# dfdazac/mpqe

Measured on AMD Instinct MI355X. Metric: query-graphs/sec (encoder fwd+bwd), higher is better.
Workload: dtype f32; 1 GPU; AIFB-shaped full query mix: 11 batches x B=512 per step (1/2/3-chain, 2x each of 2-inter, 3-inter, 3-inter_chain, 3-chain_inter), embed_dim=128, readout=mp, adaptive=True, num_layers=3 unshared, KG aifb (2601 entities, 89 typed relations); parallelism=single GPU

## Files before the change

mpqe_amd/csrc/step_chain.h:

```cpp
#pragma once
#include <type_traits>
#include "gemm_core.h"

#define CH_GB 16
#define CH_FIRST 1
#define CH_LAST 2
#define CH_LEVEL_END 4
#define CH_RELU 8
#define CH_MASK 16
#define CH_NOSTORE 32
#define CH_ADDG 64
#define CH_NOBIAS 128
#define CH_TSLOT_ON (1 << 20)
#define CH_MASK_LEVELS 4
#define CH_MAX_OPS 80
#define CH_MAX_CV 12

typedef float f32x2 __attribute__((ext_vector_type(2)));
typedef const f32x2 __attribute__((address_space(1))) * gvec2_ptr;
__device__ __forceinline__ f32x2 gload2(const float *p) { return *(gvec2_ptr)(p); }

struct ChainOp {
    unsigned char src, node, layer, level;
    int mat, flags;
    int wt_slot;
    int aux;
    int pad;
};
struct ChainRef {
    int batch, g0, fwd_begin, fwd_count, bwd_begin, bwd_count;
    int tb;
    int done;
    int e0;
    int gi0;
    int B;
    unsigned meta;
    int rof;
};

template <int NCB>
struct WHalf {
    float v[4][4][NCB];
};
template <int NCB> struct chain_vec;
template <> struct chain_vec<1> { typedef float type; };
template <> struct chain_vec<2> { typedef f32x2 type; };
template <> struct chain_vec<4> { typedef f32x4 type; };
template <int NCB> struct chain_bits { typedef unsigned char type; };
template <> struct chain_bits<4> { typedef unsigned short type; };

template <int NCB>
__device__ __forceinline__ void chain_gload(float (&d)[NCB], const float *p) {
    if constexpr (NCB == 1) d[0] = gload1(p);
    else if constexpr (NCB == 2) {
        const f32x2 q = gload2(p);
        d[0] = q[0];
        d[1] = q[1];
    } else {
        const f32x4 q = gload4(p);
#pragma unroll
        for (int c = 0; c < NCB; ++c) d[c] = q[c & 3];
    }
}
template <int NCB>
__device__ __forceinline__ void chain_store(float *p, const float (&v)[NCB]) {
    typename chain_vec<NCB>::type q;
    if constexpr (NCB == 1) q = v[0];
    else {
#pragma unroll
        for (int c = 0; c < NCB; ++c) q[c] = v[c];
    }
    *reinterpret_cast<typename chain_vec<NCB>::type *>(p) = q;
}

template <int NCB>
__device__ __forceinline__ void chain_lload(float (&d)[NCB], const float *p) {
    const typename chain_vec<NCB>::type q = *reinterpret_cast<const typename chain_vec<NCB>::type *>(p);
    if constexpr (NCB == 1) d[0] = q;
    else {
#pragma unroll
        for (int c = 0; c < NCB; ++c) d[c] = q[c];
    }
}
__device__ __forceinline__ unsigned long long chain_gran_load(const unsigned long long *g) {
#ifdef MPQE_EMU
    return *g;
#else
    typedef unsigned long long __attribute__((address_space(1))) * gp_t;
    return __hip_atomic_load((gp_t)g, __ATOMIC_RELAXED, __HIP_MEMORY_SCOPE_AGENT);
#endif
}
__device__ __forceinline__ unsigned chain_count_load(const unsigned *p) {
#ifdef MPQE_EMU
    return *p;
#else
// ... 48 lines not shown
template <int OFF>
__device__ __forceinline__ float chain_row_ror(float v) {
#ifdef MPQE_EMU
    return __shfl_xor(v, OFF, 64);
#else
    return __int_as_float(__builtin_amdgcn_update_dpp(0, __float_as_int(v), 0x120 + OFF, 0xF, 0xF, false));
#endif
}
__device__ __forceinline__ float chain_sum16(float v) {
    v += chain_row_ror<8>(v);
    v += chain_row_ror<4>(v);
    v += chain_row_ror<2>(v);
    v += chain_row_ror<1>(v);
    return v;
}
__device__ __forceinline__ void chain_relu_push(float &v, unsigned &bits) {
#ifdef MPQE_EMU
    const bool p = v > 0.f;
    v = p ? v : 0.f;
    bits = (bits << 1) | (p ? 1u : 0u);
#else
    float o;
    asm volatile("v_cmp_lt_f32 vcc, 0, %2\n\tv_cndmask_b32 %0, 0, %2, vcc\n\tv_addc_co_u32 %1, vcc, %1, %1, vcc"
                 : "=&v"(o), "+v"(bits)
                 : "v"(v)
                 : "vcc");
    v = o;
#endif
}
__device__ __forceinline__ void chain_mask_pop(float &v, unsigned &bits) {
#ifdef MPQE_EMU
    const bool p = (bits >> 31) != 0u;
    bits <<= 1;
    v = p ? v : 0.f;
#else
    float o;
    asm volatile("v_add_co_u32 %1, vcc, %1, %1\n\tv_cndmask_b32 %0, 0, %2, vcc" : "=&v"(o), "+v"(bits) : "v"(v) : "vcc");
    v = o;
#endif
}

#ifndef CHAIN_ZERO_C
#define CHAIN_ZERO_C 1
#endif
#ifndef CHAIN_DBG
#define CHAIN_DBG 0
#endif
#ifndef CHAIN_LATE_DECODE
#define CHAIN_LATE_DECODE 1
#endif
#ifndef CHAIN_NOLOAD
#define CHAIN_NOLOAD 0
#endif
template <int NCB>
__device__ __forceinline__ void chain_load_t(WHalf<NCB> &f, const float *wp, int D, int t) {
    if (CHAIN_DBG == 1) return;
#pragma unroll
    for (int u = 0; u < 4; ++u) chain_gload<NCB>(f.v[t][u], wp + (long long)(16 * t + u) * D);
}

template <int NCB>
__device__ __forceinline__ void chain_mma(f32x4 (&acc)[NCB], const WHalf<NCB> &f, const float *xp) {
#pragma unroll
    for (int t = 0; t < 4; ++t) {
        const f32x4 a = *reinterpret_cast<const f32x4 *>(xp + 16 * t);
#pragma unroll
        for (int u = 0; u < 4; ++u)
#pragma unroll
            for (int c = 0; c < NCB; ++c)
                acc[c] = __builtin_amdgcn_mfma_f32_16x16x4f32(a[u], f.v[t][u][c], acc[c], 0, 0, 0);
    }
}

template <int NCB, int KS, int NW = 4>
struct ChainLds {
    static constexpr int D = 16 * NCB * NW / KS, LDX = D + 4, BUF = 4 * CH_GB * LDX, MT = 64 * NW / KS;
    float xs[2 * BUF];
    static constexpr int NCV = CH_MAX_CV;
    float cv[NCV * D];
    typename chain_bits<NCB>::type mbits[CH_MASK_LEVELS * 4 * MT];
    const float *rowp[4 * CH_GB + 2 * CH_GB];
    float *gradp[4 * CH_GB];
    float nrm[4 * CH_GB];
    const float *wp[CH_MAX_OPS];
    int opw[CH_MAX_OPS][2];
    int opp[CH_MAX_OPS];
    int cvid[NCV];
    int cvl[NCV];
    __device__ __forceinline__ float *red() { return cv; }
#if CHAIN_DBG == 6
    long long *trace;
    int trace_n;
#endif
};

template <int NCB, int KS, int NW>
__device__ __forceinline__ void chain_colsum(ChainLds<NCB, KS, NW> &S, const float *X, unsigned mask, int ng,
                                             float *__restrict__ dst) {
    constexpr int D = 16 * NCB * NW / KS, LDX = D + 4, NP = 256 / D;
    const int col = threadIdx.x % D, part = threadIdx.x / D;
    if (threadIdx.x < 256) {
        float s = 0.f;
        for (int n = 0; n < 4; ++n) {
            if (!((mask >> n) & 1u)) continue;
            for (int i = part; i < ng; i += NP) s += X[(n * CH_GB + i) * LDX + col];
        }
        S.red()[threadIdx.x] = s;
    }
    __syncthreads();
    if (threadIdx.x < D && dst) {
        float t = S.red()[threadIdx.x];
        for (int q = 1; q < NP; ++q) t += S.red()[threadIdx.x + q * D];
        dst[threadIdx.x] = t;
    }
    __syncthreads();
}
struct ChainStep {
    int src, node, tslot, level, flags, part;
};

template <int NCB, int KS, bool BWD, int NW, bool RO = false>
__device__ __forceinline__ void chain_run(ChainLds<NCB, KS, NW> &S, const int first_op, int T , int N, int ng,
                                          float *__restrict__ Xrows, long long level_stride, int &cur,
                                          float *parts = nullptr, int blk = 0,
                                          const unsigned long long *cv_gran = nullptr, unsigned cv_tag = 0,
                                          int32_t *cv_err = nullptr) {
    constexpr int D = 16 * NCB * NW / KS, LDX = D + 4, BUF = 4 * CH_GB * LDX;
    constexpr int CW = NW / KS;
    constexpr int IPO = D / KS / 64;
    constexpr int MT = 64 * NW / KS;
    const int lane = threadIdx.x & 63, wave = threadIdx.x >> 6;
    const int j = lane & 15, kq = lane >> 4;
    const int ks = wave / CW;
    const int kbase = ks * (D / KS);
    const int colb = (wave % CW) * 16 * NCB + NCB * j;
    const bool finisher = __builtin_amdgcn_readfirstlane(ks) == KS - 1;
    auto get_op = [&](int it) -> ChainStep {
        const int k = first_op + (it < T ? it : T - 1) / IPO;
        const int w = __builtin_amdgcn_readfirstlane(S.opw[k][0]);
        ChainStep o;
        o.src = w & 0xff;
        o.node = (w >> 8) & 0xff;
        o.tslot = RO ? (w >> 16) & 0xff : o.node;
        o.level = (w >> 24) & 0xff;
        o.flags = __builtin_amdgcn_readfirstlane(S.opw[k][1]);
        o.part = __builtin_amdgcn_readfirstlane(S.opp[k]);
        return o;
    };
    struct RawOp {
        int w0, w1, w2;
    };
    auto get_raw = [&](int it) -> RawOp {
        const int k = first_op + (it < T ? it : T - 1) / IPO;
        return RawOp{S.opw[k][0], S.opw[k][1], S.opp[k]};
    };
    auto decode = [&](const RawOp &r) -> ChainStep {
        const int w = __builtin_amdgcn_readfirstlane(r.w0);
        ChainStep o;
        o.src = w & 0xff;
        o.node = (w >> 8) & 0xff;
        o.tslot = RO ? (w >> 16) & 0xff : o.node;
        o.level = (w >> 24) & 0xff;
        o.flags = __builtin_amdgcn_readfirstlane(r.w1);
        o.part = __builtin_amdgcn_readfirstlane(r.w2);
        return o;
    };
    auto wptr = [&](int it) -> const float * {
        const int itc = it < T ? it : T - 1;
        const int h = itc % IPO;
        const float *W = S.wp[first_op + itc / IPO];
        return W + (long long)(kbase + 64 * h + 4 * kq) * D + colb;
    };
    f32x4 acc[NCB];
#if CHAIN_DBG == 6
    int trace_i = BWD ? 2048 : 0;
#endif
    float bs[NCB];
#pragma unroll
    for (int c = 0; c < NCB; ++c) bs[c] = 0.f;
    const float *pend_tile = nullptr;
    float *pend_out = nullptr;
    bool pend_on = false, pend_store = false;
    int pend_part = -1;
    auto flush_rows = [&]() {
        float l[4][NCB];
#pragma unroll
        for (int r = 0; r < 4; ++r) chain_lload<NCB>(l[r], pend_tile + r * LDX);
        if (BWD) {
#pragma unroll
            for (int c = 0; c < NCB; ++c) bs[c] = 0.f;
        }
        if (ng == CH_GB) {
            if (pend_store) {
#pragma unroll
                for (int r = 0; r < 4; ++r) chain_store<NCB>(pend_out + (long long)r * N * D, l[r]);
            }
            if (BWD) {
#pragma unroll
                for (int r = 0; r < 4; ++r)
#pragma unroll
                    for (int c = 0; c < NCB; ++c) bs[c] += l[r][c];
            }
        } else {
#pragma unroll
            for (int r = 0; r < 4; ++r)
                if (4 * kq + r < ng) {
                    if (pend_store) chain_store<NCB>(pend_out + (long long)r * N * D, l[r]);
                    if (BWD) {
#pragma unroll
                        for (int c = 0; c < NCB; ++c) bs[c] += l[r][c];
                    }
                }
        }
        if (BWD && pend_part >= 0) {
            float t[NCB];
#pragma unroll
            for (int c = 0; c < NCB; ++c) {
                t[c] = bs[c] + __shfl_xor(bs[c], 16, 64);
                t[c] += __shfl_xor(t[c], 32, 64);
            }
            if (kq == 0) chain_store<NCB>(parts + (long long)(pend_part + blk) * D + colb, t);
        }
        pend_on = false;
    };
    auto item = [&](const ChainStep &op, int it, WHalf<NCB> &f, WHalf<NCB> &fn, const float *wn, auto inplace_tag) {
        constexpr bool INPLACE = decltype(inplace_tag)::value;
        const int h = it % IPO;
#if CHAIN_DBG == 6
#define CHAIN_TRACE(tag)                                                                        \
    if (S.trace && (threadIdx.x & 127) == 0 && S.trace_n < 4000) {                              \
        const long long tt_ = (long long)__builtin_amdgcn_s_memtime();                          \
        __builtin_amdgcn_s_waitcnt(0xC07F);                                                     \
        S.trace[(threadIdx.x >> 7) * 4096 + S.trace_n * 0 + trace_i] = tt_ * 8 + (tag);         \
        ++trace_i;                                                                              \
    }
        CHAIN_TRACE(0)
#else
#define CHAIN_TRACE(tag)
#endif
        const float *xp = S.xs + cur * BUF + (op.src * CH_GB + j) * LDX + kbase + 64 * h + 4 * kq;
        unsigned long long ga[RO ? 4 : 1][RO ? (NCB + 1) / 2 : 1];
        if constexpr (RO) {
            if (finisher && h == IPO - 1 && (op.flags & CH_LAST) && (op.flags & CH_ADDG)) {
                const float *Xadd = Xrows + (long long)op.level * level_stride + ((long long)(4 * kq) * N + op.node) * D + colb;
#pragma unroll
                for (int r = 0; r < 4; ++r)
#pragma unroll
                    for (int c2 = 0; c2 < (NCB + 1) / 2; ++c2) {
                        const bool in = 4 * kq + r < ng;
                        if constexpr (NCB % 2 == 0)
                            ga[r][c2] = in ? chain_gran_load(reinterpret_cast<const unsigned long long *>(Xadd + (long long)r * N * D) + c2) : 0ull;
                        else
                            ga[r][c2] = in ? (unsigned long long)chain_count_load(reinterpret_cast<const unsigned *>(Xadd + (long long)r * N * D)) : 0ull;
                    }
            }
        }
        f32x4 av[4];
#pragma unroll
        for (int t = 0; t < 4; ++t) av[t] = *reinterpret_cast<const f32x4 *>(xp + 16 * t);
#pragma unroll
        for (int t = 0; t < 4; ++t) {
            const f32x4 a = av[t];
#pragma unroll
            for (int u = 0; u < 4; ++u) {
                if (CHAIN_DBG != 1 && !CHAIN_NOLOAD && !INPLACE) chain_gload<NCB>(fn.v[t][u], wn + (long long)(16 * t + u) * D);
                __builtin_amdgcn_sched_barrier(0);
#if CHAIN_DBG == 2
#pragma unroll
                for (int c = 0; c < NCB; ++c) asm volatile("" ::"v"(f.v[t][u][c]), "v"(a[u]));
#else
                if (CHAIN_ZERO_C && t == 0 && u == 0 && h == 0 && (op.flags & CH_FIRST)) {
#pragma unroll
                    for (int c = 0; c < NCB; ++c)
                        acc[c] = __builtin_amdgcn_mfma_f32_16x16x4f32(a[u], f.v[t][u][c], f32x4{0.f, 0.f, 0.f, 0.f}, 0, 0, 0);
                } else {
#pragma unroll
                    for (int c = 0; c < NCB; ++c)
                        acc[c] = __builtin_amdgcn_mfma_f32_16x16x4f32(a[u], f.v[t][u][c], acc[c], 0, 0, 0);
                }
#endif
                __builtin_amdgcn_sched_barrier(0);
                if (CHAIN_DBG != 1 && !CHAIN_NOLOAD && INPLACE) {
                    chain_gload<NCB>(f.v[t][u], wn + (long long)(16 * t + u) * D);
                    __builtin_amdgcn_sched_barrier(0);
                }
            }
        }
        CHAIN_TRACE(1)
        if (h != IPO - 1) return;
        if (op.flags & CH_LAST) {
            static_assert(KS <= 2, "the hand-off below is written for two K parts");
            float *Xn = S.xs + (cur ^ 1) * BUF;
            float *tile = Xn + (op.tslot * CH_GB + 4 * kq) * LDX + colb;
            if (KS > 1 && !finisher) {
#pragma unroll
                for (int r = 0; r < 4; ++r) {
                    float pv[NCB];
#pragma unroll
                    for (int c = 0; c < NCB; ++c) pv[c] = acc[c][r];
                    chain_store<NCB>(tile + r * LDX, pv);
                }
            }
            float v[4][NCB];
            float bv[NCB];
            if (finisher) {
#pragma unroll
                for (int r = 0; r < 4; ++r)
#pragma unroll
                    for (int c = 0; c < NCB; ++c) v[r][c] = acc[c][r];
                if (!BWD && KS == 1) chain_lload<NCB>(bv, S.cv + op.part * D + colb);
            }
            if (KS > 1) __syncthreads();
            if (KS > 1 && finisher && !BWD) chain_lload<NCB>(bv, S.cv + op.part * D + colb);
            if (KS > 1 && !finisher) {
                if (pend_on) flush_rows();
                pend_store = !(op.flags & CH_NOSTORE);
                pend_part = op.part;
                pend_on = pend_store || (BWD && pend_part >= 0);
                pend_tile = tile;
                pend_out = Xrows + (long long)op.level * level_stride + ((long long)(4 * kq) * N + op.node) * D + colb;
                if (!BWD && cv_gran) {
                    constexpr int NCVc = ChainLds<NCB, KS, NW>::NCV;
                    const int ns = op.part + 1;
                    if (ns < NCVc && (int)threadIdx.x < D) {
                        const int id = S.cvid[ns];
                        if (id >= 0) S.cv[ns * D + threadIdx.x] = chain_gran_read1(cv_gran + (long long)id * D + threadIdx.x, cv_tag, cv_err);
                    }
                }
            }
            CHAIN_TRACE(2)
            auto finish = [&](auto mode_tag) {
                constexpr int MODE = decltype(mode_tag)::value;
                if (KS > 1) {
                    float l[4][NCB];
#pragma unroll
                    for (int r = 0; r < 4; ++r) chain_lload<NCB>(l[r], tile + r * LDX);
#pragma unroll
                    for (int r = 0; r < 4; ++r)
#pragma unroll
                        for (int c = 0; c < NCB; ++c) v[r][c] += l[r][c];
                }
                CHAIN_TRACE(4)
                const int mslot = ((op.level - 1) * 4 + op.node) * MT + (threadIdx.x & (MT - 1));
                if (!BWD && !(RO && (op.flags & CH_NOBIAS))) {
#pragma unroll
                    for (int r = 0; r < 4; ++r)
#pragma unroll
                        for (int c = 0; c < NCB; ++c) v[r][c] += bv[c];
                }
                if constexpr (RO) {
                    if (op.flags & CH_ADDG) {
#pragma unroll
                        for (int r = 0; r < 4; ++r)
#pragma unroll
                            for (int c = 0; c < NCB; ++c)
                                v[r][c] += __uint_as_float((unsigned)(ga[r][c / 2] >> (32 * (c & 1))));
                    }
                }
                if (MODE == 1) {
                    unsigned bits = 0;
#pragma unroll
                    for (int r = 0; r < 4; ++r)
// ... 9 lines not shown
                }
                CHAIN_TRACE(5)
#pragma unroll
                for (int r = 0; r < 4; ++r) chain_store<NCB>(tile + r * LDX, v[r]);
                CHAIN_TRACE(6)
                const bool var_row = KS == 1 && BWD && op.part >= 0;
                if (var_row) {
#pragma unroll
                    for (int c = 0; c < NCB; ++c) bs[c] = 0.f;
                }
                float *Xout = Xrows + (long long)op.level * level_stride + ((long long)(4 * kq) * N + op.node) * D + colb;
                if (ng == CH_GB) {
                    if (KS == 1 && !(op.flags & CH_NOSTORE)) {
#pragma unroll
                        for (int r = 0; r < 4; ++r) chain_store<NCB>(Xout + (long long)r * N * D, v[r]);
                    }
                    if (BWD && KS == 1) {
#pragma unroll
                        for (int r = 0; r < 4; ++r)
#pragma unroll
                            for (int c = 0; c < NCB; ++c) bs[c] += v[r][c];
                    }
                } else {
#pragma unroll
                    for (int r = 0; r < 4; ++r) {
                        if (4 * kq + r < ng) {
                            if (KS == 1 && !(op.flags & CH_NOSTORE)) chain_store<NCB>(Xout + (long long)r * N * D, v[r]);
                            if (BWD && KS == 1) {
#pragma unroll
                                for (int c = 0; c < NCB; ++c) bs[c] += v[r][c];
                            }
                        }
                    }
                }
                CHAIN_TRACE(7)
                if (var_row) {
                    float t[NCB];
#pragma unroll
                    for (int c = 0; c < NCB; ++c) {
                        t[c] = bs[c] + __shfl_xor(bs[c], 16, 64);
                        t[c] += __shfl_xor(t[c], 32, 64);
                    }
                    if (kq == 0) chain_store<NCB>(parts + (long long)(op.part + blk) * D + colb, t);
                }
            };
            if (finisher) {
                if (!BWD && (op.flags & CH_RELU)) finish(std::integral_constant<int, 1>());
                else if (BWD && (op.flags & CH_MASK)) finish(std::integral_constant<int, 2>());
                else finish(std::integral_constant<int, 0>());
            }
            if (!CHAIN_ZERO_C) {
#pragma unroll
                for (int c = 0; c < NCB; ++c) acc[c] = f32x4{0.f, 0.f, 0.f, 0.f};
            }
        }
        CHAIN_TRACE(3)
        if (op.flags & CH_LEVEL_END) {
            __syncthreads();
            cur ^= 1;
            if (KS > 1 && !finisher) {
                if (pend_on) flush_rows();
            }
        }
    };
    if (T <= 0) return;
#pragma unroll
    for (int c = 0; c < NCB; ++c) acc[c] = f32x4{0.f, 0.f, 0.f, 0.f};

    ChainStep oc = get_op(0), on = get_op(1);
    int it = 0;
    if constexpr (KS == 2 && CHAIN_DBG != 5) {
        WHalf<NCB> f0;
#pragma unroll
        for (int t = 0; t < 4; ++t) chain_load_t<NCB>(f0, wptr(0), D, t);
        __builtin_amdgcn_sched_barrier(0);
        const float *wn1 = wptr(1);
        while (true) {
#if CHAIN_LATE_DECODE
            const RawOp r2_ = get_raw(it + 2);
            const float *w2_ = wptr(it + 2);
            item(oc, it, f0, f0, wn1, std::true_type());
            if (++it >= T) break;
            oc = on;
            on = decode(r2_);
            wn1 = w2_;
#else
            const ChainStep o2_ = get_op(it + 2);
            const float *w2_ = wptr(it + 2);
            item(oc, it, f0, f0, wn1, std::true_type());
            if (++it >= T) break;
            oc = on;
            on = o2_;
            wn1 = w2_;
#endif
        }
    } else if constexpr (NCB <= 2) {
        WHalf<NCB> f0, f1, f2, f3;
#pragma unroll
        for (int t = 0; t < 4; ++t) chain_load_t<NCB>(f0, wptr(0), D, t);
#pragma unroll
        for (int t = 0; t < 4; ++t) chain_load_t<NCB>(f1, wptr(1), D, t);
#pragma unroll
        for (int t = 0; t < 4; ++t) chain_load_t<NCB>(f2, wptr(2), D, t);
        __builtin_amdgcn_sched_barrier(0);
#define CHAIN_STEP(F, FN)                       \
    {                                           \
        const ChainStep o2_ = get_op(it + 2);   \
        item(oc, it, F, FN, wptr(it + 3), std::false_type());      \
        if (++it >= T) break;                   \
        oc = on;                                \
        on = o2_;                               \
    }
        while (true) {
            CHAIN_STEP(f0, f3)
            CHAIN_STEP(f1, f0)
            CHAIN_STEP(f2, f1)
            CHAIN_STEP(f3, f2)
        }
#undef CHAIN_STEP
    } else {
        WHalf<NCB> f0, f1, f2;
#pragma unroll
        for (int t = 0; t < 4; ++t) chain_load_t<NCB>(f0, wptr(0), D, t);
#pragma unroll
        for (int t = 0; t < 4; ++t) chain_load_t<NCB>(f1, wptr(1), D, t);
        __builtin_amdgcn_sched_barrier(0);
#define CHAIN_STEP(F, FN)                       \
    {                                           \
        const ChainStep o2_ = get_op(it + 2);   \
        item(oc, it, F, FN, wptr(it + 2), std::false_type());      \
        if (++it >= T) break;                   \
        oc = on;                                \
        on = o2_;                               \
    }
        while (true) {
            CHAIN_STEP(f0, f2)
            CHAIN_STEP(f1, f0)
            CHAIN_STEP(f2, f1)
        }
#undef CHAIN_STEP
    }
}

struct ChainArgs {
    const ChainRef *refs;
    const ChainOp *ops;
    const long long *node_map;
    long long map_len;
    const float *mode_emb;
    long long num_modes;
    const long long *anchor_ids, *targets, *negs;
    float *H, *GH;
    const float *WT;
    const float *VT;
    unsigned *epoch_f;
    float *DG;
    const int *erow;
    long long Manchor, Gtot;
    float *parts;
    float *block_terms;
    long long level_stride;
    float margin, eps;
    float *s_pos, *s_neg, *terms;
    float *q_out;
    int32_t *err;
    int backward;
    long long *stamps;
    int cb, nchain;
    const unsigned long long *cv_gran;
    const unsigned *epoch_b;
    const unsigned *wt_count;
    int wt_blocks;
    unsigned *done;
    unsigned *arrive;
    const int *done_inc;
    int wt_early;
    int ro;
    int ro_layer, ro_scatter;
};

__device__ __forceinline__ void chain_stamp(const ChainArgs &ca, int slot) {
#ifndef MPQE_EMU
    if (ca.stamps && threadIdx.x == 0) {
        ca.stamps[(long long)ca.cb * 8 + slot] = (long long)wall_clock64();
        if (slot == 0 || slot == 6) {
            const long long t = (long long)__builtin_amdgcn_s_memtime();
            __builtin_amdgcn_s_waitcnt(0xC07F);
            ca.stamps[((long long)ca.nchain + ca.cb) * 8 + (slot == 0 ? 0 : 1)] = t;
        }
    }
#endif
}
__device__ __forceinline__ void chain_stamp_where(const ChainArgs &ca, int batch, int fwd_ops) {
#ifndef MPQE_EMU
    if (ca.stamps && threadIdx.x == 0) {
        const unsigned hw = __builtin_amdgcn_s_getreg((31 << 11) | 4);
        const unsigned xcc = __builtin_amdgcn_s_getreg((3 << 11) | 20);
        ca.stamps[(long long)ca.cb * 8 + 7] = (long long)hw | ((long long)xcc << 32) | ((long long)batch << 40) |
                                                   ((long long)fwd_ops << 48);
    }
#endif
}

template <int NCB, int KS, int NW, bool RO = false>
__device__ __forceinline__ void chain_block(const StepDev *__restrict__ sd, const LayerPtrs &lp, const TablePtrs &tabs,
                                            const ChainArgs &ca, ChainLds<NCB, KS, NW> &S) {
    constexpr int D = 16 * NCB * NW / KS, LDX = D + 4, BUF = 4 * CH_GB * LDX;
    constexpr int DB = D / 64;
    constexpr int IPO = D / KS / 64;
    constexpr int LPR = D / 4;
    const int tid = threadIdx.x, lane = tid & 63, wave = tid >> 6;
    const bool four = NW == 4 || tid < 256;
    const ChainRef ref = ca.refs[ca.cb];
    if (ref.batch < 0) return;
    const BatchDev &b = sd->b[ref.batch];
    const int N = (int)(ref.meta & 15u), A = (int)((ref.meta >> 4) & 15u), L = b.L, g0 = ref.g0;
    const int ng = ref.B - g0 < CH_GB ? ref.B - g0 : CH_GB;
    const int nrows = ng * N;
    const long long row0 = b.row_off + (long long)g0 * N;
    const long long gi0 = b.g_off + g0;

    chain_stamp(ca, 0);
    chain_stamp_where(ca, ref.batch, ref.fwd_count);
#if CHAIN_DBG == 6
#ifndef CHAIN_TRACE_BATCH
#define CHAIN_TRACE_BATCH 0
#endif
    if (threadIdx.x == 0) {
        S.trace = (ca.stamps && ref.batch == CHAIN_TRACE_BATCH && g0 == 0) ? ca.stamps + (long long)ca.nchain * 16 : nullptr;
        S.trace_n = 0;
    }
#endif
#if CHAIN_DBG == 4
    for (int q = 0; q < (int)((blockIdx.x / 8) % 4) * 6; ++q) __builtin_amdgcn_s_sleep(127);
#endif
    const int rof = RO ? ref.rof : 0, nfwd = ref.fwd_count + rof;
    const int nops = nfwd + ref.bwd_count;
    ChainOp op;
    if (tid < nops) op = ca.ops[ref.fwd_begin + tid];
    if (tid < 4 * CH_GB + 2 * CH_GB) {
        const float *src = nullptr;
        float *gdst = nullptr;
        const int rN = (int)(ref.meta & 15u), rA = (int)((ref.meta >> 4) & 15u);
        if (tid < 4 * CH_GB) {
            const int i = tid / rN, n = tid - i * rN;
            if (tid < nrows) {
                if (n < rA) {
                    const int tab = (int)((ref.meta >> (8 + 4 * n)) & 15u);
                    const long long e = (long long)ref.e0 + (long long)n * ref.B + i;
                    long long row;
                    int er = -2;
                    if (ca.erow) er = ca.erow[e];
                    if (er == -2) row = table_row(ca.node_map, ca.map_len, ca.anchor_ids[e], tabs.rows[tab], ca.err);
                    else {
                        row = er;
                        if (er < 0) flag_error(ca.err, MPQE_FLAG_BAD_NODE_ID);
                    }
                    if (row >= 0) {
                        src = tabs.table[tab] + row * D;
                        if (tabs.grad[tab]) gdst = tabs.grad[tab] + row * D;
                    }
                } else {
                    const long long m = b.var_id[n - rA];
                    if (m < 0 || m >= ca.num_modes) flag_error(ca.err, MPQE_FLAG_BAD_NODE_ID);
                    else src = ca.mode_emb + m * D;
                }
            }
            S.gradp[tid] = gdst;
        } else {
            const int i = (tid - 4 * CH_GB) & (CH_GB - 1);
            const bool is_neg = tid >= 5 * CH_GB;
            if (i < ng) {
                const int tab = (int)((ref.meta >> 20) & 15u);
                const long long e = ca.Manchor + (is_neg ? ca.Gtot : 0) + ref.gi0 + i;
                long long row;
                int er = -2;
                if (ca.erow) er = ca.erow[e];
                if (er == -2)
                    row = table_row(ca.node_map, ca.map_len, is_neg ? ca.negs[ref.gi0 + i] : ca.targets[ref.gi0 + i],
                                    tabs.rows[tab], ca.err);
                else {
                    row = er;
                    if (er < 0) flag_error(ca.err, MPQE_FLAG_BAD_NODE_ID);
                }
                if (row >= 0) src = tabs.table[tab] + row * D;
            }
        }
        S.rowp[tid] = src;
    }
    constexpr int NCV = ChainLds<NCB, KS, NW>::NCV;
    if (tid < NCV) S.cvid[tid] = -2;
    __syncthreads();
    {
        if (tid < nops) {
            if (tid < nfwd || CHAIN_DBG == 3) {
                S.wp[tid] = op.mat >= 0 ? pick_layer(lp.basis, op.layer) + (long long)op.mat * D * D
                                        : pick_layer(lp.root, op.layer);
                if (RO && (op.pad & 0xffff) > 0) S.wp[tid] = ca.WT + (long long)((op.pad & 0xffff) - 1) * D * D;
            } else {
                S.wp[tid] = ca.WT + (long long)op.wt_slot * D * D;
                if (RO && op.wt_slot < 0) S.wp[tid] = pick_layer(lp.root, op.layer);
            }
            S.opw[tid][0] = op.src | (op.node << 8) | (((RO && (op.pad & CH_TSLOT_ON)) ? (op.pad >> 16) & 15 : op.node) << 16) | (op.level << 24);
            S.opw[tid][1] = op.flags;
            S.opp[tid] = tid < nfwd ? op.wt_slot : op.aux;
            if (tid < ref.fwd_count && (op.flags & CH_LAST) && !(op.flags & CH_NOBIAS)) {
                S.cvid[op.wt_slot] = op.aux;
                S.cvl[op.wt_slot] = op.layer;
            }
        }
    }
    __syncthreads();
    chain_stamp(ca, 1);
    float wq[4] = {0.f, 0.f, 0.f, 0.f};
    auto warm = [&](int first, int count) {
        constexpr int SL = D * D / 256;
        const int slice = (g0 / CH_GB) & 7;
        const int n = count * SL;
        auto touch = [&](int item) -> float {
            const int o = item / SL, l = item - o * SL;
            return gload1(S.wp[first + o] + (long long)(slice * SL + l) * 32);
        };
#pragma unroll
        for (int k = 0; k < 4; ++k) wq[k] = touch(tid + 256 * k < n ? tid + 256 * k : 0);
        for (int item = tid + 1024; item < n; item += 256) wq[0] += touch(item);
    };

    if (four) {
        for (int f = tid; f < NCV * (D / 4); f += 256) {
            const int slot = f / (D / 4), c4 = f - slot * (D / 4);
            const int id = S.cvid[slot];
            if (id == -2 || (id >= 0 && ca.cv_gran)) continue;
            const float *src = id >= 0 ? ca.VT + (long long)id * D : pick_layer(lp.bias, S.cvl[slot]);
            *reinterpret_cast<f32x4 *>(S.cv + slot * D + 4 * c4) = src ? gload4(src + 4 * c4) : f32x4{0.f, 0.f, 0.f, 0.f};
        }
        const int nk = N * DB;
        f32x4 v[4 * DB];
#pragma unroll
        for (int k = 0; k < 4 * DB; ++k) {
            const int f = tid + 256 * (k < nk ? k : 0);
            const int r = f / (D / 4), c4 = f - r * (D / 4);
            const float *src = S.rowp[r];
            v[k] = src ? gload4(src + 4 * c4) : f32x4{0.f, 0.f, 0.f, 0.f};
        }
        if (ca.cv_gran) {
            const unsigned tag = *ca.epoch_f + 1u;
            for (int f = tid; f < (KS > 1 ? 1 : NCV) * (D / 4); f += 256) {
                const int slot = f / (D / 4), c4 = f - slot * (D / 4);
                const int id = S.cvid[slot];
                if (id < 0) continue;
                *reinterpret_cast<f32x4 *>(S.cv + slot * D + 4 * c4) =
                    chain_gran_read4(ca.cv_gran + (long long)id * D + 4 * c4, tag, ca.err);
            }
        }
        float *H0 = ca.H + row0 * D;
#pragma unroll
        for (int k = 0; k < 4 * DB; ++k) {
            const int f = tid + 256 * k;
            const int r = f / (D / 4), c4 = f - r * (D / 4);
            const int i = r / N, n = r - i * N;
            f32x4 q = v[k];
            float ss = q[0] * q[0] + q[1] * q[1] + q[2] * q[2] + q[3] * q[3];
#pragma unroll
            for (int off = LPR >> 1; off >= 16; off >>= 1) ss += __shfl_xor(ss, off, 64);
            ss = chain_sum16(ss);
            if (k < nk) {
                const bool anchor = n < A && S.rowp[r] != nullptr;
                if (anchor) {
                    const float inv = chain_rsq(ss);
                    q[0] *= inv; q[1] *= inv; q[2] *= inv; q[3] *= inv;
                    if ((f & (D / 4 - 1)) == 0) S.nrm[r] = inv;
                }
                *reinterpret_cast<f32x4 *>(S.xs + (n * CH_GB + i) * LDX + 4 * c4) = q;
                if (r < nrows) *reinterpret_cast<f32x4 *>(H0 + (long long)r * D + 4 * c4) = q;
            }
        }
    }
    __syncthreads();

    chain_stamp(ca, 2);
    constexpr int CC = D / 16;
    const int sc_i = four ? 4 * wave + (lane >> 4) : 0, sl = lane & 15;
    const float *pp_ = four ? S.rowp[4 * CH_GB + sc_i] : nullptr, *pn_ = four ? S.rowp[5 * CH_GB + sc_i] : nullptr;
    float tp[CC], tn[CC];
#pragma unroll
    for (int cc = 0; cc < CC; ++cc) {
        tp[cc] = pp_ ? gload1(pp_ + sl + 16 * cc) : 0.f;
        tn[cc] = pn_ ? gload1(pn_ + sl + 16 * cc) : 0.f;
    }
    unsigned wt_have0 = 0;
    if (tid == 0 && (ca.backward || RO) && ca.wt_count) wt_have0 = chain_count_load(ca.wt_count);
    auto wait_for_copies = [&]() {
        if (tid == 0) {
            const unsigned want = (*ca.epoch_b + 1u) * (unsigned)ca.wt_blocks;
            unsigned have = wt_have0;
            for (int spins = 0; (int)(have - want) < 0; ++spins) {
                if (spins >= (1 << 18)) {
                    flag_error(ca.err, MPQE_FLAG_INTERNAL | 0x200);
                    break;
                }
// ... 293 lines not shown
```

mpqe_amd/csrc/step_drive.h:

```cpp
#pragma once
struct StepCall {
    const mpqe_step_params_t *P;
    const mpqe_step_batch_t *B;
    int nb;
    const int64_t *anchor_ids, *targets, *negs;
    float margin;
    const mpqe_step_grads_t *G;
    int phase;
    float *loss, *scores_pos, *scores_neg;
    void *desc;
    size_t desc_bytes;
    int upload_desc;
    void *workspace;
    size_t workspace_bytes;
    int32_t *err;
    const mpqe_step_lanes_t *lanes;
    void *const *events;
    int num_events;
    void *touch, *stream;
    const mpqe_step_extra_t *extra;
};

struct StepCtx : StepCall {
    std::shared_ptr<const CachedPlan> cached;
// ... 430 lines not shown
    char *db = c.db, *wb = c.wb;
    ca.refs = at<const ChainRef>(db, hp.o_cref); ca.ops = at<const ChainOp>(db, hp.o_cops);
    ca.node_map = c.nm; ca.map_len = (long long)c.P->node_map_len;
    ca.mode_emb = c.P->mode_emb; ca.num_modes = (long long)c.P->num_modes;
    ca.anchor_ids = c.ids; ca.targets = c.tg; ca.negs = c.ng;
    ca.H = c.H; ca.GH = c.GH; ca.WT = c.WT; ca.VT = c.VT;
    ca.epoch_f = c.epoch_f; ca.epoch_b = c.epoch_b;
    ca.DG = c.use_touch ? at<float>(wb, hp.o_DG) : nullptr;
    ca.erow = c.use_touch && !c.build_touch ? reinterpret_cast<const int *>(reinterpret_cast<const char *>(c.touch) +
                                                                            touch_layout(hp.touch_M, 0).erow) : nullptr;
    ca.Manchor = (long long)hp.anchor_off[c.nb]; ca.Gtot = hp.sd.graphs_total; ca.level_stride = hp.level_stride;
    ca.parts = c.parts; ca.block_terms = at<float>(wb, hp.o_bterms);
    ca.margin = c.margin; ca.eps = 1e-8f;
    ca.s_pos = c.spos; ca.s_neg = c.sneg; ca.terms = c.terms;
    ca.q_out = c.extra ? c.extra->query_out : nullptr;
    ca.err = c.err; ca.backward = c.backward ? 1 : 0;
    ca.stamps = g_chain_stamps && 2 * hp.crefs.size() + (size_t)hp.ts_blocks <= g_chain_stamp_blocks ? g_chain_stamps : nullptr;
    ca.cb = 0; ca.nchain = pa.nchain;
    ca.cv_gran = pa.ublocks > 0 ? at<const unsigned long long>(db, hp.o_gran) : nullptr;
    ca.wt_count = pa.tblocks > 0 ? pa.wt_count : nullptr; ca.wt_blocks = wt_all;
    ca.done = c.merged ? at<unsigned>(db, hp.o_done) : nullptr;
    ca.arrive = ca.done ? ca.done + hp.done_inc.size() : nullptr; ca.done_inc = at<const int>(db, hp.o_done_inc);
    ca.ro = hp.ro_chain ? 1 : 0; ca.wt_early = hp.ro_chain && c.P->readout == MPQE_READOUT_CONCAT ? 1 : 0;
    ca.ro_layer = hp.ro_layer; ca.ro_scatter = c.P->readout_scatter;
}
static long long merged_post_args(const StepCtx &c, const PrepArgs &pa, long long zblocks, PostArgs &po) {
    const HostPlan &hp = *c.hp;
    unsigned *done = at<unsigned>(c.db, hp.o_done);
    const int zeroed = (c.P->flags & MPQE_STEP_ZERO_GRADS) ? 1 : 0;
    po.zpad = (int)((zblocks + 7) / 8 * 8);
    if (po.zpad == 0) po.zpad = 8;
    po.zmblocks = zeroed ? (int)hp.zmats.size() * c.ta.zper : 0; po.ublocks = c.ub.nops * c.ub.chunks;
    po.na = hp.post_na; po.xrank = 0;
    for (int x = 0; x < STEP_XCDS; ++x) po.xrank |= (unsigned)(hp.post_rank[x] + 1) << (4 * x);
    po.ppad = (po.zmblocks + po.ublocks + po.na - 1) / po.na * po.na;
    po.wblocks = hp.wblocks_total; po.wblock = c.ta.wblock; po.tile_n = hp.tile_n;
    po.zmats = c.ta.zmats; po.zper = c.ta.zper; po.D = c.D; po.zeroed = zeroed;
    po.ub = c.ub;
    po.ub.done = done; po.ub.done_inc = at<const int>(c.db, hp.o_done_inc); po.ub.dm = hp.dm;
    po.ub.fwd_done = pa.fwd_done; po.ub.fwd_blocks = pa.ublocks; po.ub.epoch_m = c.epoch_f + 48;
    po.slabs = c.slabs; po.H = c.H; po.GH = c.GH; po.level_stride = hp.level_stride; po.gp = c.gp;
    po.done = done; po.done_inc = po.ub.done_inc; po.epoch_m = c.epoch_f + 48;
    po.err = c.err;
    po.stamps = g_tail_stamps && (size_t)po.wblocks <= g_tail_stamp_blocks ? g_tail_stamps : nullptr;
    return pa.lead + pa.nchain + po.zpad + (long long)(po.ppad + po.wblocks + po.na - 1) / po.na * 8;
}
template <int NCB, int KS, int NW = 4, bool RO = false>
static void launch_chain_as(const StepCtx &c, dim3 grid, const ChainArgs &ca, const PrepArgs &pa, const PostArgs &po, const FinArgs &fin) {
    if (fin.count)
        hipLaunchKernelGGL((step_chain_fwd_kernel<NCB, KS, NW, RO>), grid, dim3(64 * NW), 0, c.s, c.sd, c.lp, c.tabs, ca, pa, po, fin);
    else
        hipLaunchKernelGGL((step_chain_kernel<NCB, KS, NW, RO>), grid, dim3(64 * NW), 0, c.s, c.sd, c.lp, c.tabs, ca, pa, po);
}
struct ChainDone { bool loss, reg; };
static ChainDone launch_chain(StepCtx &c, PrepArgs &pa, long long zblocks) {
    const HostPlan &hp = *c.hp;
    const int D = c.D;
    ChainDone did = {false, false};
    const int wt_all = chain_prologue(c, pa);
    ChainArgs ca;
    chain_args(c, pa, wt_all, ca);
    if (ca.stamps && c.build_touch) pa.ts.stamps = g_chain_stamps + 16 * (long long)hp.crefs.size();
    PostArgs po;
    memset(&po, 0, sizeof(po));
    long long grid_blocks = pa.lead + pa.nchain + zblocks;
    if (!c.merged && c.zero_fill && !hp.zmats.empty() && !dbg_on("ZMATS_IN_TAIL")) {
        po.zmblocks = (int)hp.zmats.size() * c.ta.zper;
        po.zmats = c.ta.zmats; po.zper = c.ta.zper; po.D = D; po.gp = c.gp;
        grid_blocks += po.zmblocks;
        c.zmats_in_chain = true;
    }
    if (c.merged) grid_blocks = merged_post_args(c, pa, zblocks, po);
    grid_blocks += pa.strail;
    dim3 cgrid((unsigned)grid_blocks);
    FinArgs fin;
    memset(&fin, 0, sizeof(fin));
    if (!c.backward && c.NL == 1 && !dbg_on("LOSS_LAUNCH")) {
        fin.count = c.epoch_f + 42; fin.epoch_f = c.epoch_f; fin.bump_b = pa.tblocks > 0 ? 1 : 0;
        fin.loss = c.loss; fin.bterms = c.bterms; fin.lm = c.lm;
        fin.notify = c.notify; fin.notify_value = c.notify_value; fin.err = c.err;
        did.loss = true;
        if (c.learned && c.extra && c.extra->readout_norms && c.P->readout_weight_decay > 0.f) {
            float wsum = 0.f;
            for (int i = 0; i < c.nb; ++i) wsum += hp.sd.b[i].weight;
            fin.reg_norms = c.extra->readout_norms; fin.reg_coef = c.P->readout_weight_decay * wsum;
            did.reg = true;
        }
    }
    mark(c, c.s);
    if (hp.ro_chain) {
        if (D == 64) launch_chain_as<1, 1, 4, true>(c, cgrid, ca, pa, po, fin);
        else if (D == 128 && (c.P->flags & MPQE_STEP_NO_KSPLIT)) launch_chain_as<2, 1, 4, true>(c, cgrid, ca, pa, po, fin);
        else if (D == 128) launch_chain_as<4, 2, 4, true>(c, cgrid, ca, pa, po, fin);
        else launch_chain_as<4, 1, 4, true>(c, cgrid, ca, pa, po, fin);
    } else if (D == 64) launch_chain_as<1, 1>(c, cgrid, ca, pa, po, fin);
    else if (D == 128 && (c.P->flags & MPQE_STEP_NO_KSPLIT)) launch_chain_as<2, 1>(c, cgrid, ca, pa, po, fin);
    else if (D == 128 && (c.P->flags & MPQE_STEP_EIGHT_WAVES)) launch_chain_as<2, 2, 8>(c, cgrid, ca, pa, po, fin);
    else if (D == 128) launch_chain_as<4, 2>(c, cgrid, ca, pa, po, fin);
    else launch_chain_as<4, 1>(c, cgrid, ca, pa, po, fin);
    mark(c, c.s);
    return did;
}
static int run_chain_form(StepCtx &c) {
    PrepArgs pa;
    memset(&pa, 0, sizeof(pa));
    long long zblocks = 0;
    if (c.zero_fill) {
        if (!c.use_touch && !c.sparse_tables) {
            ZeroSegs zt;
            memset(&zt, 0, sizeof(zt));
            long long ztb = 0;
            for (int m = 0; m < c.P->num_modes; ++m) zero_seg(zt, ztb, c.G->tables[m], (long long)c.P->table_rows[m] * c.D);
            zt.block0[zt.count] = ztb;
            if (ztb > 0) hipLaunchKernelGGL(step_zero_kernel, dim3((unsigned)ztb), dim3(256), 0, c.s, zt);
        }
        zblocks = grad_zero_segs(c, pa.zs, c.use_touch && !c.sparse_tables);
    }
    fork_lanes(c);
    const ChainDone did = launch_chain(c, pa, zblocks);
    if (!c.backward) {
        join_lanes(c);
        if (!did.loss) launch_loss(c, pa.tblocks > 0 ? 1 : 0);
        if (c.learned && !did.reg) ro_regulariser(c, false);
        return mpqe_launch_status();
    }
    mark(c, c.s);
    if (!c.merged) launch_grad_w(c, c.s);
    mark(c, c.s);
    join_lanes(c);
    launch_reduce(c);
    if (c.learned) ro_regulariser(c, true);
    return mpqe_launch_status();
}

struct LevelReadout {
    RoArgs roa;
    float *x, *gx, *h, *y, *gy, *gh;
    const float *Qc;
    float *GQc;
};
static LevelReadout level_readout(const StepCtx &c) {
    const HostPlan &hp = *c.hp;
    LevelReadout ro;
    memset(&ro, 0, sizeof(ro));
    ro.Qc = c.P->readout == MPQE_READOUT_CALLER ? at<const float>(c.wb, hp.o_Q) : nullptr;
    ro.GQc = c.P->readout == MPQE_READOUT_CALLER ? at<float>(c.wb, hp.o_GQ) : nullptr;
    ro.roa.kind = c.P->readout; ro.roa.op = c.P->readout_scatter;
    ro.roa.mrows = hp.ro_rows; ro.roa.kin = hp.ro_kin; ro.roa.level_stride = hp.level_stride;
    if (c.learned) {
// ... 175 lines not shown
```

Before: 87.12 million query-graphs/s.

## Add wide single-K-part chain form with dual accumulators and prefetched bias gran

Adds a WIDE chain configuration (NCB=2, no K split, 4 waves) that processes 128-deep K slices per item, using two independent MFMA accumulator sets summed at the end. It also prefetches the next op's bias vector from the granular cache during the current op and writes it into LDS, and skips the bulk cv warmup for that form. Launch selection gains a debug KSPLIT override, but the default still follows the existing NO_KSPLIT flag, so the new path only runs when that flag is set. The aim is longer MFMA dependency chains and less bias-load latency, paid for with more registers.

Measured after the change: 86.13 million query-graphs/s. -1.1%, worse.

```diff
diff --git a/mpqe_amd/csrc/step_chain.h b/mpqe_amd/csrc/step_chain.h
--- a/mpqe_amd/csrc/step_chain.h
+++ b/mpqe_amd/csrc/step_chain.h
@@ -38,9 +38,15 @@
     int rof;
 };
 
-template <int NCB>
+template <int NCB, int TS = 4>
 struct WHalf {
-    float v[4][4][NCB];
+    float v[TS][4][NCB];
+};
+template <int NCB, int KS, int NW>
+struct chain_form {
+    static constexpr bool WIDE = NCB == 2 && KS == 1 && NW == 4;
+    static constexpr int TS = WIDE ? 8 : 4;
+    static constexpr int IPO = 16 * NCB * NW / KS / KS / (16 * TS);
 };
 template <int NCB> struct chain_vec;
 template <> struct chain_vec<1> { typedef float type; };
@@ -195,8 +201,8 @@
 #ifndef CHAIN_NOLOAD
 #define CHAIN_NOLOAD 0
 #endif
-template <int NCB>
-__device__ __forceinline__ void chain_load_t(WHalf<NCB> &f, const float *wp, int D, int t) {
+template <int NCB, int TS>
+__device__ __forceinline__ void chain_load_t(WHalf<NCB, TS> &f, const float *wp, int D, int t) {
     if (CHAIN_DBG == 1) return;
 #pragma unroll
     for (int u = 0; u < 4; ++u) chain_gload<NCB>(f.v[t][u], wp + (long long)(16 * t + u) * D);
@@ -260,6 +266,7 @@
 }
 struct ChainStep {
     int src, node, tslot, level, flags, part;
+    int nid;
 };
 
 template <int NCB, int KS, bool BWD, int NW, bool RO = false>
@@ -270,7 +277,10 @@
                                           int32_t *cv_err = nullptr) {
     constexpr int D = 16 * NCB * NW / KS, LDX = D + 4, BUF = 4 * CH_GB * LDX;
     constexpr int CW = NW / KS;
-    constexpr int IPO = D / KS / 64;
+    constexpr bool WIDE = chain_form<NCB, KS, NW>::WIDE;
+    constexpr int TS = chain_form<NCB, KS, NW>::TS;
+    constexpr int IPO = chain_form<NCB, KS, NW>::IPO;
+    typedef WHalf<NCB, TS> WBuf;
     constexpr int MT = 64 * NW / KS;
     const int lane = threadIdx.x & 63, wave = threadIdx.x >> 6;
     const int j = lane & 15, kq = lane >> 4;
@@ -278,17 +288,25 @@
     const int kbase = ks * (D / KS);
     const int colb = (wave % CW) * 16 * NCB + NCB * j;
     const bool finisher = __builtin_amdgcn_readfirstlane(ks) == KS - 1;
-    auto get_op = [&](int it) -> ChainStep {
-        const int k = first_op + (it < T ? it : T - 1) / IPO;
-        const int w = __builtin_amdgcn_readfirstlane(S.opw[k][0]);
+    auto unpack = [&](int w0, int w1, int w2) -> ChainStep {
+        const int w = __builtin_amdgcn_readfirstlane(w0);
         ChainStep o;
         o.src = w & 0xff;
         o.node = (w >> 8) & 0xff;
         o.tslot = RO ? (w >> 16) & 0xff : o.node;
         o.level = (w >> 24) & 0xff;
-        o.flags = __builtin_amdgcn_readfirstlane(S.opw[k][1]);
-        o.part = __builtin_amdgcn_readfirstlane(S.opp[k]);
+        o.flags = __builtin_amdgcn_readfirstlane(w1);
+        o.part = __builtin_amdgcn_readfirstlane(w2);
+        o.nid = 0;
+        if (WIDE && !BWD) {
+            o.nid = o.part >> 8;
+            o.part &= 0xff;
+        }
         return o;
+    };
+    auto get_op = [&](int it) -> ChainStep {
+        const int k = first_op + (it < T ? it : T - 1) / IPO;
+        return unpack(S.opw[k][0], S.opw[k][1], S.opp[k]);
     };
     struct RawOp {
         int w0, w1, w2;
@@ -297,24 +315,15 @@
         const int k = first_op + (it < T ? it : T - 1) / IPO;
         return RawOp{S.opw[k][0], S.opw[k][1], S.opp[k]};
     };
-    auto decode = [&](const RawOp &r) -> ChainStep {
-        const int w = __builtin_amdgcn_readfirstlane(r.w0);
-        ChainStep o;
-        o.src = w & 0xff;
-        o.node = (w >> 8) & 0xff;
-        o.tslot = RO ? (w >> 16) & 0xff : o.node;
-        o.level = (w >> 24) & 0xff;
-        o.flags = __builtin_amdgcn_readfirstlane(r.w1);
-        o.part = __builtin_amdgcn_readfirstlane(r.w2);
-        return o;
-    };
+    auto decode = [&](const RawOp &r) -> ChainStep { return unpack(r.w0, r.w1, r.w2); };
     auto wptr = [&](int it) -> const float * {
         const int itc = it < T ? it : T - 1;
         const int h = itc % IPO;
         const float *W = S.wp[first_op + itc / IPO];
-        return W + (long long)(kbase + 64 * h + 4 * kq) * D + colb;
+        return W + (long long)(kbase + 16 * TS * h + 4 * kq) * D + colb;
     };
     f32x4 acc[NCB];
+    f32x4 acc1[WIDE ? NCB : 1];
 #if CHAIN_DBG == 6
     int trace_i = BWD ? 2048 : 0;
 #endif
@@ -366,7 +375,7 @@
         }
         pend_on = false;
     };
-    auto item = [&](const ChainStep &op, int it, WHalf<NCB> &f, WHalf<NCB> &fn, const float *wn, auto inplace_tag) {
+    auto item = [&](const ChainStep &op, int it, WBuf &f, WBuf &fn, const float *wn, auto inplace_tag) {
         constexpr bool INPLACE = decltype(inplace_tag)::value;
         const int h = it % IPO;
 #if CHAIN_DBG == 6
@@ -381,7 +390,7 @@
 #else
 #define CHAIN_TRACE(tag)
 #endif
-        const float *xp = S.xs + cur * BUF + (op.src * CH_GB + j) * LDX + kbase + 64 * h + 4 * kq;
+        const float *xp = S.xs + cur * BUF + (op.src * CH_GB + j) * LDX + kbase + 16 * TS * h + 4 * kq;
         unsigned long long ga[RO ? 4 : 1][RO ? (NCB + 1) / 2 : 1];
         if constexpr (RO) {
             if (finisher && h == IPO - 1 && (op.flags & CH_LAST) && (op.flags & CH_ADDG)) {
@@ -398,11 +407,20 @@
                     }
             }
         }
-        f32x4 av[4];
-#pragma unroll
-        for (int t = 0; t < 4; ++t) av[t] = *reinterpret_cast<const f32x4 *>(xp + 16 * t);
-#pragma unroll
-        for (int t = 0; t < 4; ++t) {
+        unsigned long long cg[WIDE && !BWD ? NCB : 1];
+        const unsigned long long *cgp = nullptr;
+        bool cv_next = false;
+        if constexpr (WIDE && !BWD) {
+            cv_next = cv_gran && h == IPO - 1 && (op.flags & CH_LAST) && op.nid > 0;
+            cgp = cv_next ? cv_gran + (long long)(op.nid - 1) * D + colb : reinterpret_cast<const unsigned long long *>(Xrows) + (colb >> 1);
+#pragma unroll
+            for (int c = 0; c < NCB; ++c) cg[c] = chain_gran_load(cgp + (cv_next ? c : 0));
+        }
+        f32x4 av[TS];
+#pragma unroll
+        for (int t = 0; t < TS; ++t) av[t] = *reinterpret_cast<const f32x4 *>(xp + 16 * t);
+#pragma unroll
+        for (int t = 0; t < TS; ++t) {
             const f32x4 a = av[t];
 #pragma unroll
             for (int u = 0; u < 4; ++u) {
@@ -412,14 +430,15 @@
 #pragma unroll
                 for (int c = 0; c < NCB; ++c) asm volatile("" ::"v"(f.v[t][u][c]), "v"(a[u]));
 #else
-                if (CHAIN_ZERO_C && t == 0 && u == 0 && h == 0 && (op.flags & CH_FIRST)) {
+                f32x4 *ap = WIDE && t >= TS / 2 ? acc1 : acc;
+                if (CHAIN_ZERO_C && (t == 0 || (WIDE && t == TS / 2)) && u == 0 && h == 0 && (op.flags & CH_FIRST)) {
 #pragma unroll
                     for (int c = 0; c < NCB; ++c)
-                        acc[c] = __builtin_amdgcn_mfma_f32_16x16x4f32(a[u], f.v[t][u][c], f32x4{0.f, 0.f, 0.f, 0.f}, 0, 0, 0);
+                        ap[c] = __builtin_amdgcn_mfma_f32_16x16x4f32(a[u], f.v[t][u][c], f32x4{0.f, 0.f, 0.f, 0.f}, 0, 0, 0);
                 } else {
 #pragma unroll
                     for (int c = 0; c < NCB; ++c)
-                        acc[c] = __builtin_amdgcn_mfma_f32_16x16x4f32(a[u], f.v[t][u][c], acc[c], 0, 0, 0);
+                        ap[c] = __builtin_amdgcn_mfma_f32_16x16x4f32(a[u], f.v[t][u][c], ap[c], 0, 0, 0);
                 }
 #endif
                 __builtin_amdgcn_sched_barrier(0);
@@ -430,6 +449,15 @@
             }
         }
         CHAIN_TRACE(1)
+        if constexpr (WIDE && !BWD) {
+            if (cv_next) {
+                float cvv[NCB];
+#pragma unroll
+                for (int c = 0; c < NCB; ++c)
+                    cvv[c] = (unsigned)(cg[c] >> 32) == cv_tag ? __uint_as_float((unsigned)cg[c]) : chain_gran_read1(cgp + c, cv_tag, cv_err);
+                chain_store<NCB>(S.cv + (op.part + 1) * D + colb, cvv);
+            }
+        }
         if (h != IPO - 1) return;
         if (op.flags & CH_LAST) {
             static_assert(KS <= 2, "the hand-off below is written for two K parts");
@@ -450,7 +478,7 @@
 #pragma unroll
                 for (int r = 0; r < 4; ++r)
 #pragma unroll
-                    for (int c = 0; c < NCB; ++c) v[r][c] = acc[c][r];
+                    for (int c = 0; c < NCB; ++c) v[r][c] = WIDE ? acc1[c][r] + acc[c][r] : acc[c][r];
                 if (!BWD && KS == 1) chain_lload<NCB>(bv, S.cv + op.part * D + colb);
             }
             if (KS > 1) __syncthreads();
@@ -566,6 +594,8 @@
             if (!CHAIN_ZERO_C) {
 #pragma unroll
                 for (int c = 0; c < NCB; ++c) acc[c] = f32x4{0.f, 0.f, 0.f, 0.f};
+#pragma unroll
+                for (int c = 0; c < (WIDE ? NCB : 1); ++c) acc1[c] = f32x4{0.f, 0.f, 0.f, 0.f};
             }
         }
         CHAIN_TRACE(3)
@@ -580,13 +610,15 @@
     if (T <= 0) return;
 #pragma unroll
     for (int c = 0; c < NCB; ++c) acc[c] = f32x4{0.f, 0.f, 0.f, 0.f};
+#pragma unroll
+    for (int c = 0; c < (WIDE ? NCB : 1); ++c) acc1[c] = f32x4{0.f, 0.f, 0.f, 0.f};
 
     ChainStep oc = get_op(0), on = get_op(1);
     int it = 0;
-    if constexpr (KS == 2 && CHAIN_DBG != 5) {
-        WHalf<NCB> f0;
-#pragma unroll
-        for (int t = 0; t < 4; ++t) chain_load_t<NCB>(f0, wptr(0), D, t);
+    if constexpr ((KS == 2 || WIDE) && CHAIN_DBG != 5) {
+        WBuf f0;
+#pragma unroll
+        for (int t = 0; t < TS; ++t) chain_load_t<NCB, TS>(f0, wptr(0), D, t);
         __builtin_amdgcn_sched_barrier(0);
         const float *wn1 = wptr(1);
         while (true) {
@@ -609,13 +641,13 @@
 #endif
         }
     } else if constexpr (NCB <= 2) {
-        WHalf<NCB> f0, f1, f2, f3;
-#pragma unroll
-        for (int t = 0; t < 4; ++t) chain_load_t<NCB>(f0, wptr(0), D, t);
-#pragma unroll
-        for (int t = 0; t < 4; ++t) chain_load_t<NCB>(f1, wptr(1), D, t);
-#pragma unroll
-        for (int t = 0; t < 4; ++t) chain_load_t<NCB>(f2, wptr(2), D, t);
+        WBuf f0, f1, f2, f3;
+#pragma unroll
+        for (int t = 0; t < 4; ++t) chain_load_t<NCB, TS>(f0, wptr(0), D, t);
+#pragma unroll
+        for (int t = 0; t < 4; ++t) chain_load_t<NCB, TS>(f1, wptr(1), D, t);
+#pragma unroll
+        for (int t = 0; t < 4; ++t) chain_load_t<NCB, TS>(f2, wptr(2), D, t);
         __builtin_amdgcn_sched_barrier(0);
 #define CHAIN_STEP(F, FN)                       \
     {                                           \
@@ -633,11 +665,11 @@
         }
 #undef CHAIN_STEP
     } else {
-        WHalf<NCB> f0, f1, f2;
-#pragma unroll
-        for (int t = 0; t < 4; ++t) chain_load_t<NCB>(f0, wptr(0), D, t);
-#pragma unroll
-        for (int t = 0; t < 4; ++t) chain_load_t<NCB>(f1, wptr(1), D, t);
+        WBuf f0, f1, f2;
+#pragma unroll
+        for (int t = 0; t < 4; ++t) chain_load_t<NCB, TS>(f0, wptr(0), D, t);
+#pragma unroll
+        for (int t = 0; t < 4; ++t) chain_load_t<NCB, TS>(f1, wptr(1), D, t);
         __builtin_amdgcn_sched_barrier(0);
 #define CHAIN_STEP(F, FN)                       \
     {                                           \
@@ -721,7 +753,8 @@
                                             const ChainArgs &ca, ChainLds<NCB, KS, NW> &S) {
     constexpr int D = 16 * NCB * NW / KS, LDX = D + 4, BUF = 4 * CH_GB * LDX;
     constexpr int DB = D / 64;
-    constexpr int IPO = D / KS / 64;
+    constexpr int IPO = chain_form<NCB, KS, NW>::IPO;
+    constexpr bool WIDE = chain_form<NCB, KS, NW>::WIDE;
     constexpr int LPR = D / 4;
     const int tid = threadIdx.x, lane = tid & 63, wave = tid >> 6;
     const bool four = NW == 4 || tid < 256;
@@ -825,6 +858,13 @@
         }
     }
     __syncthreads();
+    if constexpr (WIDE) {
+        if (tid < ref.fwd_count && (op.flags & CH_LAST) && !(op.flags & CH_NOBIAS) && ca.cv_gran) {
+            const int ns = op.wt_slot + 1;
+            const int id = ns < NCV ? S.cvid[ns] : -1;
+            if (id >= 0) S.opp[tid] = op.wt_slot | ((id + 1) << 8);
+        }
+    }
     chain_stamp(ca, 1);
     float wq[4] = {0.f, 0.f, 0.f, 0.f};
     auto warm = [&](int first, int count) {
@@ -859,7 +899,7 @@
         }
         if (ca.cv_gran) {
             const unsigned tag = *ca.epoch_f + 1u;
-            for (int f = tid; f < (KS > 1 ? 1 : NCV) * (D / 4); f += 256) {
+            for (int f = tid; f < (KS > 1 || WIDE ? 1 : NCV) * (D / 4); f += 256) {
                 const int slot = f / (D / 4), c4 = f - slot * (D / 4);
                 const int id = S.cvid[slot];
                 if (id < 0) continue;
diff --git a/mpqe_amd/csrc/step_drive.h b/mpqe_amd/csrc/step_drive.h
--- a/mpqe_amd/csrc/step_drive.h
+++ b/mpqe_amd/csrc/step_drive.h
@@ -506,6 +506,7 @@
     else
         hipLaunchKernelGGL((step_chain_kernel<NCB, KS, NW, RO>), grid, dim3(64 * NW), 0, c.s, c.sd, c.lp, c.tabs, ca, pa, po);
 }
+static bool chain_unsplit_default(const StepCtx &c) { return (c.P->flags & MPQE_STEP_NO_KSPLIT) != 0; }
 struct ChainDone { bool loss, reg; };
 static ChainDone launch_chain(StepCtx &c, PrepArgs &pa, long long zblocks) {
     const HostPlan &hp = *c.hp;
@@ -542,13 +543,15 @@
         }
     }
     mark(c, c.s);
+    const int ksplit_opt = mpqe_dbg_value("KSPLIT", -1);
+    const bool unsplit = ksplit_opt >= 0 ? ksplit_opt == 0 : chain_unsplit_default(c);
     if (hp.ro_chain) {
         if (D == 64) launch_chain_as<1, 1, 4, true>(c, cgrid, ca, pa, po, fin);
-        else if (D == 128 && (c.P->flags & MPQE_STEP_NO_KSPLIT)) launch_chain_as<2, 1, 4, true>(c, cgrid, ca, pa, po, fin);
+        else if (D == 128 && unsplit) launch_chain_as<2, 1, 4, true>(c, cgrid, ca, pa, po, fin);
         else if (D == 128) launch_chain_as<4, 2, 4, true>(c, cgrid, ca, pa, po, fin);
         else launch_chain_as<4, 1, 4, true>(c, cgrid, ca, pa, po, fin);
     } else if (D == 64) launch_chain_as<1, 1>(c, cgrid, ca, pa, po, fin);
-    else if (D == 128 && (c.P->flags & MPQE_STEP_NO_KSPLIT)) launch_chain_as<2, 1>(c, cgrid, ca, pa, po, fin);
+    else if (D == 128 && unsplit) launch_chain_as<2, 1>(c, cgrid, ca, pa, po, fin);
     else if (D == 128 && (c.P->flags & MPQE_STEP_EIGHT_WAVES)) launch_chain_as<2, 2, 8>(c, cgrid, ca, pa, po, fin);
     else if (D == 128) launch_chain_as<4, 2>(c, cgrid, ca, pa, po, fin);
     else launch_chain_as<4, 1>(c, cgrid, ca, pa, po, fin);
```
